# alekseyzimin/PacBio

Measured on NVIDIA B200. Metric: pacbio_bases_aligned_per_s, higher is better.
Workload: dtype int64+f64

## Files before the change

pacbio_b200/csrc/align.cu:

```cuda
#include "align.cuh"
#include "group.cuh"

#include <algorithm>
#include <cmath>
#include <cstdlib>
#include <cstring>
#include <memory>

namespace {

static int setup_final_rows(mr_context* ctx, mr_workspace& ws, uint64_t Sc, coords_soa& fin) {
  memset(&fin, 0, sizeof(fin));
  MR_TRY(ws.fin_i32.ensure(ctx, Sc * 4 * 5)); MR_TRY(ws.fin_u32.ensure(ctx, Sc * 4 * 8)); MR_TRY(ws.fin_f64.ensure(ctx, Sc * 8 * 3));
  MR_TRY(ws.fin_u64.ensure(ctx, Sc * 8 * 3)); MR_TRY(ws.fin_u8.ensure(ctx, Sc * 2));
  { int32_t* b = ws.fin_i32.as<int32_t>(); fin.rs = b; fin.re = b + Sc; fin.qs = b + 2 * Sc; fin.qe = b + 3 * Sc; fin.nb_mers = b + 4 * Sc; }
  { uint32_t* b = ws.fin_u32.as<uint32_t>(); fin.pb_cons = b; fin.sr_cons = b + Sc; fin.pb_cover = b + 2 * Sc; fin.sr_cover = b + 3 * Sc;
    fin.ql = b + 4 * Sc; fin.sr = b + 5 * Sc; fin.read = b + 6 * Sc; fin.info_len = b + 7 * Sc; }
  { double* b = ws.fin_f64.as<double>(); fin.stretch = b; fin.offset = b + Sc; fin.avg_err = b + 2 * Sc; }
  { uint64_t* b = ws.fin_u64.as<uint64_t>(); fin.info_off = b; fin.chain_pos = b + Sc; }
  { uint8_t* b = ws.fin_u8.as<uint8_t>(); fin.rn = b; fin.use_bwd = b + Sc; }
  return MR_OK;
}

static int setup_graph_nodes(mr_context* ctx, mr_workspace& ws, uint64_t Sc, graph_args& GA) {
// ... 370 lines not shown
    }
    if(kMulti || sz) __stcs(rec + g0 + j, out);
    __stcs(size + g0 + j, sz);
    if((!kMulti || (part_flags & 2)) && sz) ++nlist;
  }
  if(kMulti && !(part_flags & 1)) nlook = 0;
  nlook = __reduce_add_sync(MR_FULL_MASK, nlook); ntail = __reduce_add_sync(MR_FULL_MASK, ntail);
  nlist = __reduce_add_sync(MR_FULL_MASK, nlist); nbucket = __reduce_add_sync(MR_FULL_MASK, nbucket);
  if((threadIdx.x & 31) == 0) {
    if(nlook) atomicAdd(&looked, nlook);
    if(ntail) atomicAdd(&scanned, ntail);
    if(nlist) atomicAdd(&listed, nlist);
    if(nbucket) atomicAdd(&buckets, nbucket);
  }
  __syncthreads();
  if(threadIdx.x == 0) {
    if(looked) atomicAdd(n_lookups, (unsigned long long)looked);
    if(scanned) atomicAdd(n_tails, (unsigned long long)scanned);
    if(listed) atomicAdd(n_lists, (unsigned long long)listed);
    if(buckets) atomicAdd(n_buckets, (unsigned long long)buckets);
  }
}

__global__ void __launch_bounds__(256) read_threshold_kernel(const uint64_t* __restrict__ read_start, uint32_t nbits,
                                                              uint32_t* __restrict__ size, uint32_t* __restrict__ thr_out) {
  __shared__ uint32_t hist[2048];
  __shared__ uint64_t sw[8];
  __shared__ uint32_t sh_bin, sh_before, sh_count;
  const uint32_t r = blockIdx.x;
  const uint64_t rs = read_start[r];
  const uint32_t rlen = (uint32_t)(read_start[r + 1] - rs);
  uint32_t* sz = size + rs;
  if(threadIdx.x == 0) sh_count = 0;
  __syncthreads();
  uint32_t mine = 0;
  for(uint32_t i = threadIdx.x; i < rlen; i += 256) mine += sz[i] != 0;
  if(mine) atomicAdd(&sh_count, mine);
  __syncthreads();
  const uint32_t L = sh_count;
  const double   scaled = (double)L * 0.99;
  const uint32_t sum_thresh = (uint32_t)round(scaled);
  if(L == 0 || sum_thresh >= L) { if(threadIdx.x == 0) thr_out[r] = 0xffffffffu; return; }
  uint32_t kth = sum_thresh + 1, prefix = 0, remaining = nbits;
  while(remaining > 0) {
    const uint32_t d = remaining < 11 ? remaining : 11, shift = remaining - d;
    for(int i = threadIdx.x; i < 2048; i += 256) hist[i] = 0;
    __syncthreads();
    for(uint32_t i = threadIdx.x; i < rlen; i += 256) {
      const uint32_t v = sz[i];
      if(v != 0 && (remaining >= 32 || (v >> remaining) == prefix)) atomicAdd(&hist[(v >> shift) & ((1u << d) - 1)], 1u);
    }
    __syncthreads();
    uint32_t local[8], s = 0;
#pragma unroll
    for(int j = 0; j < 8; ++j) { local[j] = hist[threadIdx.x * 8 + j]; s += local[j]; }
    uint64_t total;
    uint32_t before = (uint32_t)prim::block_exclusive_scan_256(s, sw, total);
    if(before < kth && kth <= before + s) {
#pragma unroll
      for(int j = 0; j < 8; ++j) {
        if(kth <= before + local[j]) { sh_bin = threadIdx.x * 8 + j; sh_before = before; break; }
        before += local[j];
      }
    }
    __syncthreads();
    kth -= sh_before;
    prefix = (prefix << d) | sh_bin;
    remaining = shift;
    __syncthreads();
  }
  if(threadIdx.x == 0) thr_out[r] = prefix;
  for(uint32_t i = threadIdx.x; i < rlen; i += 256) if(sz[i] > prefix) sz[i] = 0;
}

__device__ __forceinline__ void emit_hit(const index_view& iv, uint32_t read, uint32_t pb_off, uint32_t sa_rank, bool minus,
                                         uint64_t slot, uint64_t* __restrict__ keys, uint64_t* __restrict__ pays,
                                         uint32_t& n_bad) {
  uint32_t sr, off;
  bool inside;
  if(iv.saloc) {
    const uint2 l = __ldg(iv.saloc + sa_rank);
    sr = l.x; off = l.y;
    inside = sr != 0xffffffffu;
  } else inside = index_locate(iv, __ldg(iv.sa + sa_rank), sr, off);
  if(inside) {
    const int32_t soff = minus ? -(int32_t)off : (int32_t)off;
    keys[slot] = ((uint64_t)read << 32) | (iv.sr_base + sr);
    pays[slot] = (uint64_t)pb_off | ((uint64_t)(uint32_t)soff << 32);
  } else {
    keys[slot] = ((uint64_t)read << 32) | iv.nseq_all;
    pays[slot] = 0;
    ++n_bad;
  }
}

__global__ void __launch_bounds__(kSeedThreads) tile_hits_kernel(const uint64_t* __restrict__ read_start,
                                                                  const uint32_t* __restrict__ tile_read, const uint32_t* __restrict__ tile_pos,
                                                                  const uint32_t* __restrict__ size, uint32_t* __restrict__ tile_hits,
                                                                  unsigned long long* __restrict__ overflow) {
  __shared__ uint64_t sw[8];
  const uint32_t r = tile_read[blockIdx.x];
  const uint64_t rs = read_start[r];
  const uint32_t rlen = (uint32_t)(read_start[r + 1] - rs);
  const uint32_t tpos = tile_pos[blockIdx.x];
  uint32_t s = 0;
#pragma unroll
  for(int it = 0; it < kTile / kSeedThreads; ++it) {
    const uint32_t pos = tpos + it * kSeedThreads + threadIdx.x;
    if(pos < rlen) s += __ldcs(size + rs + pos);
  }
  uint64_t total;
  (void)prim::block_exclusive_scan_256(s, sw, total);
  if(threadIdx.x == 0) {
    tile_hits[blockIdx.x] = total > 0xffffffffULL ? 0xffffffffu : (uint32_t)total;
    if(total > 0xffffffffULL) atomicAdd(overflow, 1ULL);
  }
}

template<bool kMulti>
__global__ void __launch_bounds__(kSeedThreads) expand_kernel(index_view iv, const index_view* __restrict__ more_views, uint32_t nparts,
                                                               uint64_t rec_stride, const uint64_t* __restrict__ read_start,
                                                               const uint32_t* __restrict__ tile_read, const uint32_t* __restrict__ tile_pos,
                                                               const uint4* __restrict__ rec, const uint32_t* __restrict__ size,
                                                               const uint64_t* __restrict__ tile_off,
                                                               uint64_t* __restrict__ keys, uint64_t* __restrict__ pays,
                                                               unsigned long long* __restrict__ n_invalid) {
  __shared__ uint64_t sw[8];
  __shared__ uint32_t s_off[kSeedThreads];
  __shared__ uint4    s_rec[kSeedThreads];
  uint64_t run = tile_off[blockIdx.x];
  if(tile_off[blockIdx.x + 1] == run) return;
  const uint32_t r = tile_read[blockIdx.x];
  const uint64_t rs = read_start[r];
  const uint32_t rlen = (uint32_t)(read_start[r + 1] - rs);
  const uint32_t tpos = tile_pos[blockIdx.x];
  uint32_t n_bad = 0;
  for(int it = 0; it < kTile / kSeedThreads; ++it) {
    const uint32_t pos = tpos + it * kSeedThreads + threadIdx.x;
    uint32_t sz = 0;
    uint4 rc = make_uint4(0, 0, 0, 0);
    if(pos < rlen) {
      sz = __ldcs(size + rs + pos);
      if(sz) rc = __ldcs(rec + rs + pos);
    }
    uint64_t in_iter;
    s_off[threadIdx.x] = (uint32_t)prim::block_exclusive_scan_256(sz, sw, in_iter);
    s_rec[threadIdx.x] = rc;
    __syncthreads();
    for(uint32_t h = threadIdx.x; h < (uint32_t)in_iter; h += kSeedThreads) {
      uint32_t lo = 0, hi = kSeedThreads;
      while(hi - lo > 1) { const uint32_t mid = (lo + hi) >> 1; if(s_off[mid] <= h) lo = mid; else hi = mid; }
      uint4 c = s_rec[lo];
      uint32_t j = h - s_off[lo];
      if(kMulti) {
        uint32_t part = 0;
        while(j >= c.y + c.w && part + 1 < nparts) {
          j -= c.y + c.w;
          ++part;
          c = __ldg(rec + part * rec_stride + rs + tpos + it * kSeedThreads + lo);
        }
        const bool minus = j >= c.y;
        emit_hit(part ? more_views[part - 1] : iv, r, tpos + it * kSeedThreads + lo + 1, minus ? c.z + (j - c.y) : c.x + j, minus,
                 run + h, keys, pays, n_bad);
        continue;
      }
      const bool minus = j >= c.y;
      emit_hit(iv, r, tpos + it * kSeedThreads + lo + 1, minus ? c.z + (j - c.y) : c.x + j, minus, run + h, keys, pays, n_bad);
    }
    run += in_iter;
    __syncthreads();
  }
  if(n_bad) atomicAdd(n_invalid, (unsigned long long)n_bad);
}

__global__ void __launch_bounds__(256) fine_windows_kernel(uint64_t S, survivors sv, const uint64_t* __restrict__ read_start, uint32_t kk,
                                                            uint64_t* __restrict__ wkey, uint32_t* __restrict__ wrow,
                                                            double* __restrict__ wbegin, double* __restrict__ wend,
                                                            uint32_t* __restrict__ gread, uint32_t* __restrict__ gsr, uint32_t* __restrict__ giter) {
  const uint64_t i = (uint64_t)blockIdx.x * blockDim.x + threadIdx.x;
  if(i >= S) return;
  const uint32_t read = sv.read[i], sr = sv.sr[i];
  const double stretch = sv.stretch[i], offset = sv.offset[i], err = sv.avg_err[i];
  const double rl = (double)(read_start[read + 1] - read_start[read]);
  const double s1 = stretch + offset;
  wbegin[i] = fmax(0.0, s1 - err);
  const double t = stretch * (double)sv.ql[i];
  const double e1 = t + offset;
  const double e2 = e1 + err;
  wend[i] = fmin(rl, e2 - (double)kk);
  wkey[i] = ((uint64_t)read << 32) | sr;
  wrow[i] = (uint32_t)i;
  gread[i] = read; gsr[i] = sr; giter[i] = sv.iter[i];
}

__global__ void __launch_bounds__(kSeedThreads) fine_seed_kernel(index_view iv, bool first_part, uint32_t kk, packed_reads bases,
// ... 556 lines not shown
    typedef void (*seed_fn)(index_view, uint32_t, packed_reads, const uint64_t*, const uint32_t*, const uint32_t*, const uint32_t*, uint32_t,
                            uint4*, uint32_t*, unsigned long long*, unsigned long long*, unsigned long long*, unsigned long long*);
    auto pick = [](bool multi, const index_view& v) -> seed_fn {
      const bool nibs = v.nib != nullptr, bytes = v.tail_bytes == 1;
      if(multi) return nibs ? (bytes ? seed_lookup_kernel<true, true, true> : seed_lookup_kernel<true, true, false>)
                            : (bytes ? seed_lookup_kernel<true, false, true> : seed_lookup_kernel<true, false, false>);
      return nibs ? (bytes ? seed_lookup_kernel<false, true, true> : seed_lookup_kernel<false, true, false>)
                  : (bytes ? seed_lookup_kernel<false, false, true> : seed_lookup_kernel<false, false, false>);
    };
    for(uint32_t part = 0; part < nparts; ++part) {
      l2_window(ctx, st, part ? idx->more[part - 1] : idx, true);
      const index_view& pv = idx->part_view(part);
      pick(nparts > 1, pv)<<<ntiles, kSeedThreads, 0, st>>>(pv, nparts == 1 ? 3u : ((part == 0 ? 1u : 0u) | (part + 1 == nparts ? 2u : 0u)),
                                                           d_bases, d_read_start, ws.tile_read.as<uint32_t>(), ws.tile_pos.as<uint32_t>(),
                                                           ws.tile_tbase.as<uint32_t>(), p->max_count > 0 ? (uint32_t)p->max_count : 0u,
                                                           ws.rec.as<uint4>() + part * rec_stride, ws.size.as<uint32_t>(), ctr + 0, ctr + 6, ctr + 9, ctr + 10);
      MR_LAUNCHED(ctx);
    }
    l2_window(ctx, st, idx, false);
    timer.next("count threshold");
    uint32_t nbits = 32;
    if(p->max_count > 1) { nbits = 0; while((1u << nbits) < (uint32_t)p->max_count) ++nbits; }
    else if(p->max_count == 1) nbits = 1;
    read_threshold_kernel<<<nreads, 256, 0, st>>>(d_read_start, nbits, ws.size.as<uint32_t>(), ws.thr.as<uint32_t>());
    MR_LAUNCHED(ctx);
  }
  timer.next("hit expansion");
  if(ntiles) {
    tile_hits_kernel<<<ntiles, kSeedThreads, 0, st>>>(d_read_start, ws.tile_read.as<uint32_t>(), ws.tile_pos.as<uint32_t>(),
                                                     ws.size.as<uint32_t>(), ws.tile_cand.as<uint32_t>(), ctr + 11);
    MR_LAUNCHED(ctx);
  }
  MR_TRY((prim::exclusive_scan<prim::ptr_in_u32, uint64_t>(ctx, prim::ptr_in_u32{ ws.tile_cand.as<uint32_t>() }, ntiles, ws.hit_off.as<uint64_t>(),
                                                           ws.scan_scratch, (uint64_t*)(ctr + 1))));
  if(ntiles) MR_CUDA(ctx, cudaMemcpyAsync(ws.hit_off.as<uint64_t>() + ntiles, ctr + 1, sizeof(uint64_t), cudaMemcpyDeviceToDevice, st));
  int sr_bits = 1;
  while((1ULL << sr_bits) <= (uint64_t)iv.nseq_all) ++sr_bits;
  MR_CUDA(ctx, cudaMemcpyAsync(h_ctr, ctr, 12 * sizeof(uint64_t), cudaMemcpyDeviceToHost, st));
  MR_CUDA(ctx, ctx->wait(st));
  if(h_ctr[11]) return ctx->fail(MR_ELIMIT, "mr_align_batch: 2^32 or more hits in one 1024-base tile; use --max-count");
  const uint64_t H = h_ctr[1];
  MR_TRACE_MSG("batch: %u reads, %llu bases, %llu lookups, %llu raw hits", nreads, (unsigned long long)T, (unsigned long long)h_ctr[0], (unsigned long long)H);
  res->view.n_kmers_looked_up = h_ctr[0];
  res->view.n_tail_entries = h_ctr[6];
  res->view.n_lists = h_ctr[9];
  res->view.n_buckets = h_ctr[10];
  static const uint64_t hit_limit = getenv("MR_MAX_HITS") ? strtoull(getenv("MR_MAX_HITS"), nullptr, 0) : (1ULL << 32);
  if(H >= hit_limit) return ctx->fail(MR_ELIMIT, "mr_align_batch: too many hits in one batch; use smaller batches");

  uint64_t G = 0, S = 0, cap = 0;
  const bool taps = ctx->keep_taps;
  uint64_t *skeys = nullptr, *spays = nullptr;
  chain_args A;
  memset(&A, 0, sizeof(A));
  if(H) {
    MR_TRY(ws.key0.ensure(ctx, (H + 2) * 8)); MR_TRY(ws.key1.ensure(ctx, (H + 2) * 8));
    MR_TRY(ws.pay0.ensure(ctx, (H + 2) * 8)); MR_TRY(ws.pay1.ensure(ctx, (H + 2) * 8));
    if(nparts == 1)
      expand_kernel<false><<<ntiles, kSeedThreads, 0, st>>>(iv, nullptr, 1, 0, d_read_start, ws.tile_read.as<uint32_t>(), ws.tile_pos.as<uint32_t>(),
                                                          ws.rec.as<uint4>(), ws.size.as<uint32_t>(), ws.hit_off.as<uint64_t>(),
                                                          ws.key0.as<uint64_t>(), ws.pay0.as<uint64_t>(), ctr + 2);
    else
      expand_kernel<true><<<ntiles, kSeedThreads, 0, st>>>(iv, idx->more_views.as<index_view>(), nparts, rec_stride, d_read_start,
                                                         ws.tile_read.as<uint32_t>(), ws.tile_pos.as<uint32_t>(),
                                                         ws.rec.as<uint4>(), ws.size.as<uint32_t>(), ws.hit_off.as<uint64_t>(),
                                                         ws.key0.as<uint64_t>(), ws.pay0.as<uint64_t>(), ctr + 2);
    MR_LAUNCHED(ctx);
    timer.next("group sort");
    static const bool read_sort_on = !(getenv("MR_READ_SORT") && atoi(getenv("MR_READ_SORT")) == 0);
    const bool read_sort = read_sort_on && group_sort_usable(sr_bits);
    uint64_t *alt_key, *alt_pay;
    if(read_sort) {
      MR_TRY(ws.head.ensure(ctx, H + 2));
      group_sort_args GS;
      GS.keys_in = ws.key0.as<uint64_t>(); GS.pays_in = ws.pay0.as<uint64_t>();
      GS.keys_out = ws.key1.as<uint64_t>(); GS.pays_out = ws.pay1.as<uint64_t>();
      GS.head = ws.head.as<uint8_t>(); GS.hit_off = ws.hit_off.as<uint64_t>(); GS.tile_first = ws.tile_first.as<uint32_t>();
      GS.nseq_all = iv.nseq_all; GS.sr_bits = sr_bits; GS.n_invalid_groups = ctr + 14; GS.cap = 0; GS.idx_bits = 0;
      MR_TRY(launch_group_sort(ctx, GS, nreads));
      skeys = GS.keys_out; spays = GS.pays_out; alt_key = GS.keys_in; alt_pay = GS.pays_in;
      MR_TRY((prim::flag_count<head_byte>(ctx, head_byte{ GS.head }, H, ws.scan_scratch, (uint64_t*)(ctr + 3))));
    } else {
      bool in_first = true;
      MR_TRY((prim::radix_sort_pairs<uint64_t, uint64_t>(ctx, ws.key0.as<uint64_t>(), ws.pay0.as<uint64_t>(), ws.key1.as<uint64_t>(),
                                                         ws.pay1.as<uint64_t>(), H, 0, sr_bits, ws.sort, &in_first)));
      skeys = in_first ? ws.key0.as<uint64_t>() : ws.key1.as<uint64_t>();
      spays = in_first ? ws.pay0.as<uint64_t>() : ws.pay1.as<uint64_t>();
      alt_key = in_first ? ws.key1.as<uint64_t>() : ws.key0.as<uint64_t>();
      alt_pay = in_first ? ws.pay1.as<uint64_t>() : ws.pay0.as<uint64_t>();
      MR_TRY((prim::flag_count<head_flag>(ctx, head_flag{ skeys, iv.nseq_all }, H, ws.scan_scratch, (uint64_t*)(ctr + 3))));
    }
    MR_CUDA(ctx, cudaMemcpyAsync(h_ctr, ctr, 16 * sizeof(uint64_t), cudaMemcpyDeviceToHost, st));
    MR_CUDA(ctx, ctx->wait(st));
    G = h_ctr[3];
    MR_TRACE_MSG("sorted (%s); %llu groups", read_sort ? "per read" : "device-wide", (unsigned long long)G);
    const uint64_t Hvalid = H - h_ctr[2];
    res->view.n_hits = Hvalid;
    res->view.n_groups = G - (read_sort ? h_ctr[14] : 0);
    MR_TRY(ws.group_start.ensure(ctx, (G + 2) * 8));
    if(read_sort) {
      MR_TRY((prim::flag_positions<head_byte>(ctx, head_byte{ ws.head.as<uint8_t>() }, H, ws.scan_scratch, ws.group_start.as<uint64_t>())));
      MR_CUDA(ctx, cudaMemcpyAsync(ws.group_start.as<uint64_t>() + G, ctr + 1, 8, cudaMemcpyDeviceToDevice, st));
// ... 563 lines not shown
```

pacbio_b200/csrc/align.cuh:

```cuda
#pragma once
#include <algorithm>
#include <cstdlib>
#include "index.cuh"
#include "primitives.cuh"

#include <mutex>

constexpr int      kTile        = 1024;
constexpr int      kSeedThreads = 256;
constexpr uint32_t kNone        = 0xffffffffu;

struct packed_reads {
  const uint64_t* __restrict__ codes;
  const uint64_t* __restrict__ nmask;
  int tma;
};

struct coords_soa {
  int32_t  *rs, *re, *qs, *qe, *nb_mers;
  uint32_t *pb_cons, *sr_cons, *pb_cover, *sr_cover, *ql, *sr, *read;
  uint8_t  *rn, *use_bwd;
  double   *stretch, *offset, *avg_err;
  uint64_t *info_off;
  uint32_t *info_len;
  uint64_t *chain_pos;
};

struct fine_buffers {
  dev_buf wkey0, wkey1, wrow0, wrow1, wbegin, wend, gread, gsr, giter, table_off, row_cnt, group_start;
  prim::sort_scratch sort;
};

struct mr_staged {
// ... 118 lines not shown
```

pacbio_b200/csrc/group.cu:

```cuda
#include "align.cuh"
#include "group.cuh"

namespace {

constexpr int kGsRounds  = 16;
constexpr int kGsDigit   = 7;
constexpr int kGsRadix   = 1 << kGsDigit;
constexpr int kFbRounds  = 4;

template<int kThreads>
struct gs_layout {
  static constexpr int kWarps = kThreads / 32;
  static constexpr int kCap   = kThreads * kGsRounds;
  static constexpr size_t pay_off = 0;
  static constexpr size_t arr_off = pay_off + (size_t)(kCap + 2) * 8;
  static constexpr size_t cnt_off = arr_off + (size_t)kCap * 4;
  static constexpr size_t tot_off = cnt_off + (size_t)kWarps * kGsRadix * 4;
  static constexpr size_t dbs_off = tot_off + kGsRadix * 4;
  static constexpr size_t bsz_off = dbs_off + kGsRadix * 4;
  static constexpr size_t bst_off = bsz_off + kGsRadix * 4;
  static constexpr size_t wsm_off = bst_off + kGsRadix * 4;
  static constexpr size_t cbs_off = wsm_off + 16;
  static constexpr size_t bar_off = cbs_off + kGsRadix * 4;
  static constexpr size_t bytes   = bar_off + 32;
// ... 59 lines not shown
  uint32_t run = 0, inc = 0;
  if(threadIdx.x < kGsRadix) {
#pragma unroll 8
    for(int w = 0; w < kWarps; ++w) { const uint32_t t = cnt[w][threadIdx.x]; cnt[w][threadIdx.x] = run; run += t; }
    tot[threadIdx.x] = run;
    if(kScan) {
      inc = run;
#pragma unroll
      for(int s = 1; s < 32; s <<= 1) { const uint32_t o = __shfl_up_sync(MR_FULL_MASK, inc, s); if(lane >= (unsigned)s) inc += o; }
      if(lane == 31) wsum[warp] = inc;
    }
  }
  __syncthreads();
  if(kScan) {
    if(threadIdx.x < kGsRadix) {
      uint32_t before = 0;
      for(unsigned w = 0; w < warp; ++w) before += wsum[w];
      dbase[threadIdx.x] = before + inc - run;
    }
    __syncthreads();
  }
}

template<int kThreads, bool kMatch>
__device__ void sort_range_smem(const uint64_t* kin, const uint64_t* pin, uint64_t* ko, uint64_t* po, uint8_t* head,
                                uint32_t n, uint32_t key_base, int key_bits, uint32_t ib, uint64_t rhi, uint32_t& phase) {
  typedef gs_sm<kThreads> Sm;
  constexpr int kWarps = kThreads / 32;
  const unsigned warp = threadIdx.x >> 5, lt = lanemask_lt();
  uint32_t* arr = Sm::arr();
  const uint32_t skew = (uint32_t)(((uintptr_t)pin >> 3) & 1u);
  if(threadIdx.x == 0) {
    const uint32_t bytes = ((n + skew + 1) & ~1u) * 8u;
    mbar_expect_tx(Sm::bar(), bytes);
    bulk_copy_g2s(Sm::spay(), pin - skew, bytes, Sm::bar());
  }
#pragma unroll 4
  for(uint32_t j = threadIdx.x; j < n; j += kThreads) arr[j] = (((uint32_t)kin[j] - key_base) << ib) | j;
  __syncthreads();
  const uint32_t R = (n + kThreads - 1) / kThreads;
  const uint32_t piece = warp * 32 * R + (threadIdx.x & 31);
  const int passes = (key_bits + kGsDigit - 1) / kGsDigit;
  for(int p = 0; p < passes; ++p) {
    const int shift = (int)ib + p * kGsDigit;
    for(int i = threadIdx.x; i < kWarps * kGsRadix; i += kThreads) (&Sm::cnt()[0][0])[i] = 0;
    __syncthreads();
    uint32_t e[kGsRounds], rk[kGsRounds / 2];
#pragma unroll
    for(int i = 0; i < kGsRounds; ++i) {
      if((i & 1) == 0) rk[i >> 1] = 0;
      if((uint32_t)i < R) {
        const uint32_t pos = piece + i * 32;
        const bool valid = pos < n;
        e[i] = valid ? arr[pos] : 0u;
        rk[i >> 1] |= rank_round<kMatch>(valid ? (e[i] >> shift) & (kGsRadix - 1) : (uint32_t)kGsRadix, Sm::cnt()[warp], lt) << (16 * (i & 1));
      }
    }
    __syncthreads();
    digit_prefix<kWarps, true>(Sm::cnt(), Sm::tot(), Sm::dbase(), Sm::wsum());
#pragma unroll
    for(int i = 0; i < kGsRounds; ++i) {
      if((uint32_t)i < R && piece + i * 32 < n) {
        const uint32_t d = (e[i] >> shift) & (kGsRadix - 1);
        arr[Sm::dbase()[d] + Sm::cnt()[warp][d] + ((rk[i >> 1] >> (16 * (i & 1))) & 0xffffu)] = e[i];
      }
    }
    __syncthreads();
  }
  mbar_wait(Sm::bar(), phase & 1u);
  ++phase;
  const uint32_t imask = (1u << ib) - 1;
#pragma unroll 4
  for(uint32_t j = threadIdx.x; j < n; j += kThreads) {
    const uint32_t x = arr[j], rel = x >> ib;
    ko[j] = rhi | (uint64_t)(key_base + rel);
    po[j] = Sm::spay()[skew + (x & imask)];
    head[j] = j == 0 || (arr[j - 1] >> ib) != rel;
  }
  __syncthreads();
}

template<int kThreads, bool kMatch>
__device__ void radix_pass_global(const uint64_t* sk, const uint64_t* sp, uint64_t* dk, uint64_t* dp, uint32_t n,
                                  int shift, uint32_t dmask, bool keep, uint32_t& gc) {
  typedef gs_sm<kThreads> Sm;
  constexpr int kWarps = kThreads / 32, kChunk = kThreads * kFbRounds;
  const unsigned lane = threadIdx.x & 31, warp = threadIdx.x >> 5, lt = lanemask_lt();
  uint32_t *tot = Sm::tot(), *gbase = Sm::dbase(), *cbase = Sm::cbase();
  uint16_t (*C)[kWarps][kGsRadix] = reinterpret_cast<uint16_t (*)[kWarps][kGsRadix]>(Sm::cnt());
  for(int i = threadIdx.x; i < kGsRadix; i += kThreads) tot[i] = 0;
  for(int i = threadIdx.x; i < kWarps * kGsRadix; i += kThreads) (&C[0][0][0])[i] = 0;
  asm volatile("fence.proxy.async;" ::: "memory");
  __syncthreads();
// ... 77 lines not shown
__device__ void sort_range_global(uint64_t* ak, uint64_t* ap, uint64_t* bk, uint64_t* bp, uint8_t* head,
                                  uint32_t n, int bits, bool stay, uint32_t& gc) {
  int passes = (bits + kGsDigit - 1) / kGsDigit;
  if(((passes & 1) == 0) != stay) ++passes;
  if(passes) {
    const int width = max(1, (bits + passes - 1) / passes);
    for(int p = 0; p < passes; ++p) {
      radix_pass_global<kThreads, kMatch>(ak, ap, bk, bp, n, p * width, (1u << width) - 1, false, gc);
      uint64_t* t = ak; ak = bk; bk = t;
      t = ap; ap = bp; bp = t;
    }
  }
  for(uint32_t j = threadIdx.x; j < n; j += kThreads) head[j] = j == 0 || (uint32_t)ak[j] != (uint32_t)ak[j - 1];
  __syncthreads();
}

template<int kThreads, bool kMatch>
__global__ void __launch_bounds__(kThreads, kThreads == 1024 ? 1 : 2) group_sort_kernel(group_sort_args A) {
  typedef gs_sm<kThreads> Sm;

  const uint32_t r = blockIdx.x;
  const uint64_t seg = A.hit_off[A.tile_first[r]];
  const uint64_t n64 = A.hit_off[A.tile_first[r + 1]] - seg;
  if(n64 == 0) return;
  const uint32_t n = (uint32_t)n64;
  const uint64_t rhi = (uint64_t)r << 32;
  uint32_t phase = 0, gc = 0;
  if(threadIdx.x == 0) { mbar_init(Sm::bar(), 1); mbar_init(Sm::cbar(), 1); mbar_init(Sm::cbar() + 1, 1); mbar_init(Sm::cbar() + 2, 1); }
  __syncthreads();
  uint64_t *kin = A.keys_in + seg, *pin = A.pays_in + seg, *ko = A.keys_out + seg, *po = A.pays_out + seg;
  uint8_t* head = A.head + seg;

  if(n <= A.cap) {
    sort_range_smem<kThreads, kMatch>(kin, pin, ko, po, head, n, 0u, A.sr_bits, A.idx_bits, rhi, phase);
  } else {
    const int low_bits = A.sr_bits > kGsDigit ? A.sr_bits - kGsDigit : 0;
    if(low_bits + (int)A.range_idx_bits > 32) {
      sort_range_global<kThreads, kMatch>(kin, pin, ko, po, head, n, A.sr_bits, false, gc);
    } else {
      radix_pass_global<kThreads, kMatch>(kin, pin, ko, po, n, low_bits, kGsRadix - 1, true, gc);
      asm volatile("fence.proxy.async;" ::: "memory");
      __syncthreads();
      const uint32_t rcap = A.range_cap;
      uint32_t b = 0;
      while(b < (uint32_t)kGsRadix) {
        const uint32_t sz = Sm::bsize()[b];
        if(sz == 0) { ++b; continue; }
        const uint32_t at = Sm::bstart()[b];
        if(sz > rcap) {
          sort_range_global<kThreads, kMatch>(ko + at, po + at, kin + at, pin + at, head + at, sz, low_bits, true, gc);
          asm volatile("fence.proxy.async;" ::: "memory");
          __syncthreads();
          ++b;
          continue;
        }
        uint32_t b1 = b + 1, total = sz;
        while(b1 < (uint32_t)kGsRadix) {
          const uint32_t nb = b1 + 1 - b;
          const int kb = low_bits + (32 - __clz(nb - 1));
          if(total + Sm::bsize()[b1] > rcap || kb + (int)A.range_idx_bits > 32) break;
          total += Sm::bsize()[b1];
          ++b1;
        }
        const uint32_t nb = b1 - b;
        const int kb = low_bits + (nb > 1 ? 32 - __clz(nb - 1) : 0);
        sort_range_smem<kThreads, kMatch>(ko + at, po + at, ko + at, po + at, head + at, total, b << low_bits, kb, A.range_idx_bits, rhi, phase);
        b = b1;
      }
    }
  }
  if(threadIdx.x == 0 && (uint32_t)ko[n - 1] == A.nseq_all) atomicAdd(A.n_invalid_groups, 1ULL);
}

}

int group_sort_threads() {
  static const int v = [] { const char* e = getenv("MR_GSORT_THREADS"); const int x = e ? atoi(e) : 0; return x == 1024 ? 1024 : 512; }();
  return v;
}

static int group_sort_cap_bits() {
  static const int env_bits = [] { const char* e = getenv("MR_GSORT_CAP"); int x = e ? atoi(e) : 0, b = 0; while((2 << b) <= x) ++b; return x >= 32 ? b : 31; }();
  return std::min(group_sort_threads() == 1024 ? 14 : 13, env_bits);
}

bool group_sort_usable(int sr_bits) {
  return std::max(0, sr_bits - kGsDigit) + group_sort_cap_bits() <= 32;
}

int launch_group_sort(mr_context* ctx, group_sort_args A, uint32_t nreads) {
  if(!nreads) return MR_OK;
  const int cb = group_sort_cap_bits();
  A.range_idx_bits = (uint32_t)cb; A.range_cap = 1u << cb;
  A.idx_bits = (uint32_t)std::max(0, std::min(cb, 32 - A.sr_bits));
  A.cap = A.sr_bits + 5 <= 32 ? 1u << A.idx_bits : 0u;
  typedef void (*kernel_t)(group_sort_args);
  const bool wide = group_sort_threads() == 1024;
  const kernel_t fn = wide ? (g_gs_match ? group_sort_kernel<1024, true> : group_sort_kernel<1024, false>)
                           : (g_gs_match ? group_sort_kernel<512, true> : group_sort_kernel<512, false>);
  const size_t smem = wide ? gs_layout<1024>::bytes : gs_layout<512>::bytes;
  MR_CUDA(ctx, cudaFuncSetAttribute(fn, cudaFuncAttributeMaxDynamicSharedMemorySize, (int)smem));
  fn<<<nreads, wide ? 1024 : 512, smem, ctx->stream>>>(A);
  MR_LAUNCHED(ctx);
  return MR_OK;
}
```

pacbio_b200/csrc/group.cuh:

```cuda
#pragma once
#include "common.cuh"

struct group_sort_args {
  uint64_t* keys_in;  uint64_t* pays_in;
  uint64_t* keys_out; uint64_t* pays_out;
  uint8_t*  head;
  const uint64_t* hit_off;
  const uint32_t* tile_first;
  uint32_t nseq_all;
  int      sr_bits;
  unsigned long long* n_invalid_groups;
  uint32_t cap, idx_bits, range_cap, range_idx_bits;
};

bool group_sort_usable(int sr_bits);
int launch_group_sort(mr_context* ctx, group_sort_args A, uint32_t nreads);
```

Measured before the change: 9.770 billion.

## Fuse hit expansion into per-read group sort and fold tile counts into thresholding

Tile hit counting moves into read_threshold_kernel, which now zeroes over-threshold sizes and writes per-tile totals plus a per-read max in the same pass, so the separate tile_hits_kernel goes away. For reads whose hit count fits the in-shared-memory cap, a new expand_group_kernel expands hits directly into shared memory and sorts them there, skipping the global key/pay write and re-read. The old expand_kernel and group_sort_kernel now run only for oversized reads, gated on a host-read max counter. This adds more kernel variants and shared-memory pressure, and the per-read loop in the threshold kernel serialises tile scans.

```diff
diff --git a/pacbio_b200/csrc/align.cu b/pacbio_b200/csrc/align.cu
--- a/pacbio_b200/csrc/align.cu
+++ b/pacbio_b200/csrc/align.cu
@@ -416,8 +416,10 @@
   }
 }
 
-__global__ void __launch_bounds__(256) read_threshold_kernel(const uint64_t* __restrict__ read_start, uint32_t nbits,
-                                                              uint32_t* __restrict__ size, uint32_t* __restrict__ thr_out) {
+__global__ void __launch_bounds__(256) read_threshold_kernel(const uint64_t* __restrict__ read_start, const uint32_t* __restrict__ tile_first,
+                                                              uint32_t nbits, uint32_t* __restrict__ size, uint32_t* __restrict__ thr_out,
+                                                              uint32_t* __restrict__ tile_hits, unsigned long long* __restrict__ overflow,
+                                                              unsigned long long* __restrict__ max_hits) {
   __shared__ uint32_t hist[2048];
   __shared__ uint64_t sw[8];
   __shared__ uint32_t sh_bin, sh_before, sh_count;
@@ -434,108 +436,87 @@
   const uint32_t L = sh_count;
   const double   scaled = (double)L * 0.99;
   const uint32_t sum_thresh = (uint32_t)round(scaled);
-  if(L == 0 || sum_thresh >= L) { if(threadIdx.x == 0) thr_out[r] = 0xffffffffu; return; }
-  uint32_t kth = sum_thresh + 1, prefix = 0, remaining = nbits;
-  while(remaining > 0) {
-    const uint32_t d = remaining < 11 ? remaining : 11, shift = remaining - d;
-    for(int i = threadIdx.x; i < 2048; i += 256) hist[i] = 0;
-    __syncthreads();
-    for(uint32_t i = threadIdx.x; i < rlen; i += 256) {
-      const uint32_t v = sz[i];
-      if(v != 0 && (remaining >= 32 || (v >> remaining) == prefix)) atomicAdd(&hist[(v >> shift) & ((1u << d) - 1)], 1u);
-    }
-    __syncthreads();
-    uint32_t local[8], s = 0;
+  uint32_t prefix = 0xffffffffu;
+  if(L != 0 && sum_thresh < L) {
+    uint32_t kth = sum_thresh + 1, remaining = nbits;
+    prefix = 0;
+    while(remaining > 0) {
+      const uint32_t d = remaining < 11 ? remaining : 11, shift = remaining - d;
+      for(int i = threadIdx.x; i < 2048; i += 256) hist[i] = 0;
+      __syncthreads();
+      for(uint32_t i = threadIdx.x; i < rlen; i += 256) {
+        const uint32_t v = sz[i];
+        if(v != 0 && (remaining >= 32 || (v >> remaining) == prefix)) atomicAdd(&hist[(v >> shift) & ((1u << d) - 1)], 1u);
+      }
+      __syncthreads();
+      uint32_t local[8], s = 0;
 #pragma unroll
-    for(int j = 0; j < 8; ++j) { local[j] = hist[threadIdx.x * 8 + j]; s += local[j]; }
+      for(int j = 0; j < 8; ++j) { local[j] = hist[threadIdx.x * 8 + j]; s += local[j]; }
+      uint64_t total;
+      uint32_t before = (uint32_t)prim::block_exclusive_scan_256(s, sw, total);
+      if(before < kth && kth <= before + s) {
+#pragma unroll
+        for(int j = 0; j < 8; ++j) {
+          if(kth <= before + local[j]) { sh_bin = threadIdx.x * 8 + j; sh_before = before; break; }
+          before += local[j];
+        }
+      }
+      __syncthreads();
+      kth -= sh_before;
+      prefix = (prefix << d) | sh_bin;
+      remaining = shift;
+      __syncthreads();
+    }
+  }
+  if(threadIdx.x == 0) thr_out[r] = prefix;
+  const uint32_t t0 = tile_first[r], nt = tile_first[r + 1] - t0;
+  uint64_t read_hits = 0;
+  for(uint32_t t = 0; t < nt; ++t) {
+    uint64_t s = 0;
+#pragma unroll
+    for(int it = 0; it < kTile / 256; ++it) {
+      const uint32_t i = t * kTile + it * 256 + threadIdx.x;
+      if(i < rlen) {
+        const uint32_t v = sz[i];
+        if(v > prefix) sz[i] = 0;
+        else s += v;
+      }
+    }
     uint64_t total;
-    uint32_t before = (uint32_t)prim::block_exclusive_scan_256(s, sw, total);
-    if(before < kth && kth <= before + s) {
-#pragma unroll
-      for(int j = 0; j < 8; ++j) {
-        if(kth <= before + local[j]) { sh_bin = threadIdx.x * 8 + j; sh_before = before; break; }
-        before += local[j];
-      }
-    }
-    __syncthreads();
-    kth -= sh_before;
-    prefix = (prefix << d) | sh_bin;
-    remaining = shift;
-    __syncthreads();
-  }
-  if(threadIdx.x == 0) thr_out[r] = prefix;
-  for(uint32_t i = threadIdx.x; i < rlen; i += 256) if(sz[i] > prefix) sz[i] = 0;
-}
-
-__device__ __forceinline__ void emit_hit(const index_view& iv, uint32_t read, uint32_t pb_off, uint32_t sa_rank, bool minus,
-                                         uint64_t slot, uint64_t* __restrict__ keys, uint64_t* __restrict__ pays,
-                                         uint32_t& n_bad) {
-  uint32_t sr, off;
-  bool inside;
-  if(iv.saloc) {
-    const uint2 l = __ldg(iv.saloc + sa_rank);
-    sr = l.x; off = l.y;
-    inside = sr != 0xffffffffu;
-  } else inside = index_locate(iv, __ldg(iv.sa + sa_rank), sr, off);
-  if(inside) {
-    const int32_t soff = minus ? -(int32_t)off : (int32_t)off;
-    keys[slot] = ((uint64_t)read << 32) | (iv.sr_base + sr);
-    pays[slot] = (uint64_t)pb_off | ((uint64_t)(uint32_t)soff << 32);
-  } else {
-    keys[slot] = ((uint64_t)read << 32) | iv.nseq_all;
-    pays[slot] = 0;
-    ++n_bad;
-  }
-}
-
-__global__ void __launch_bounds__(kSeedThreads) tile_hits_kernel(const uint64_t* __restrict__ read_start,
-                                                                  const uint32_t* __restrict__ tile_read, const uint32_t* __restrict__ tile_pos,
-                                                                  const uint32_t* __restrict__ size, uint32_t* __restrict__ tile_hits,
-                                                                  unsigned long long* __restrict__ overflow) {
-  __shared__ uint64_t sw[8];
-  const uint32_t r = tile_read[blockIdx.x];
-  const uint64_t rs = read_start[r];
-  const uint32_t rlen = (uint32_t)(read_start[r + 1] - rs);
-  const uint32_t tpos = tile_pos[blockIdx.x];
-  uint32_t s = 0;
-#pragma unroll
-  for(int it = 0; it < kTile / kSeedThreads; ++it) {
-    const uint32_t pos = tpos + it * kSeedThreads + threadIdx.x;
-    if(pos < rlen) s += __ldcs(size + rs + pos);
-  }
-  uint64_t total;
-  (void)prim::block_exclusive_scan_256(s, sw, total);
-  if(threadIdx.x == 0) {
-    tile_hits[blockIdx.x] = total > 0xffffffffULL ? 0xffffffffu : (uint32_t)total;
-    if(total > 0xffffffffULL) atomicAdd(overflow, 1ULL);
-  }
+    (void)prim::block_exclusive_scan_256(s, sw, total);
+    read_hits += total;
+    if(threadIdx.x == 0) {
+      tile_hits[t0 + t] = total > 0xffffffffULL ? 0xffffffffu : (uint32_t)total;
+      if(total > 0xffffffffULL) atomicAdd(overflow, 1ULL);
+    }
+  }
+  if(threadIdx.x == 0 && read_hits) atomicMax(max_hits, (unsigned long long)read_hits);
 }
 
 template<bool kMulti>
-__global__ void __launch_bounds__(kSeedThreads) expand_kernel(index_view iv, const index_view* __restrict__ more_views, uint32_t nparts,
-                                                               uint64_t rec_stride, const uint64_t* __restrict__ read_start,
+__global__ void __launch_bounds__(kSeedThreads) expand_kernel(hit_lists L, const uint32_t* __restrict__ tile_first, uint32_t cap,
                                                                const uint32_t* __restrict__ tile_read, const uint32_t* __restrict__ tile_pos,
-                                                               const uint4* __restrict__ rec, const uint32_t* __restrict__ size,
                                                                const uint64_t* __restrict__ tile_off,
-                                                               uint64_t* __restrict__ keys, uint64_t* __restrict__ pays,
-                                                               unsigned long long* __restrict__ n_invalid) {
+                                                               uint64_t* __restrict__ keys, uint64_t* __restrict__ pays) {
   __shared__ uint64_t sw[8];
   __shared__ uint32_t s_off[kSeedThreads];
   __shared__ uint4    s_rec[kSeedThreads];
   uint64_t run = tile_off[blockIdx.x];
   if(tile_off[blockIdx.x + 1] == run) return;
   const uint32_t r = tile_read[blockIdx.x];
-  const uint64_t rs = read_start[r];
-  const uint32_t rlen = (uint32_t)(read_start[r + 1] - rs);
+  if(tile_off[tile_first[r + 1]] - tile_off[tile_first[r]] <= cap) return;
+  const uint64_t rs = L.read_start[r];
+  const uint32_t rlen = (uint32_t)(L.read_start[r + 1] - rs);
   const uint32_t tpos = tile_pos[blockIdx.x];
+  const uint64_t khi = (uint64_t)r << 32;
   uint32_t n_bad = 0;
   for(int it = 0; it < kTile / kSeedThreads; ++it) {
     const uint32_t pos = tpos + it * kSeedThreads + threadIdx.x;
     uint32_t sz = 0;
     uint4 rc = make_uint4(0, 0, 0, 0);
     if(pos < rlen) {
-      sz = __ldcs(size + rs + pos);
-      if(sz) rc = __ldcs(rec + rs + pos);
+      sz = __ldcs(L.size + rs + pos);
+      if(sz) rc = __ldcs(L.rec + rs + pos);
     }
     uint64_t in_iter;
     s_off[threadIdx.x] = (uint32_t)prim::block_exclusive_scan_256(sz, sw, in_iter);
@@ -544,27 +525,24 @@
     for(uint32_t h = threadIdx.x; h < (uint32_t)in_iter; h += kSeedThreads) {
       uint32_t lo = 0, hi = kSeedThreads;
       while(hi - lo > 1) { const uint32_t mid = (lo + hi) >> 1; if(s_off[mid] <= h) lo = mid; else hi = mid; }
-      uint4 c = s_rec[lo];
-      uint32_t j = h - s_off[lo];
-      if(kMulti) {
-        uint32_t part = 0;
-        while(j >= c.y + c.w && part + 1 < nparts) {
-          j -= c.y + c.w;
-          ++part;
-          c = __ldg(rec + part * rec_stride + rs + tpos + it * kSeedThreads + lo);
-        }
-        const bool minus = j >= c.y;
-        emit_hit(part ? more_views[part - 1] : iv, r, tpos + it * kSeedThreads + lo + 1, minus ? c.z + (j - c.y) : c.x + j, minus,
-                 run + h, keys, pays, n_bad);
-        continue;
+      const uint32_t at = tpos + it * kSeedThreads + lo;
+      bool minus;
+      uint32_t part, sr;
+      uint64_t pay;
+      const uint32_t rank = list_entry<kMulti>(L, rs + at, s_rec[lo], h - s_off[lo], minus, part);
+      if(locate_hit(part ? L.more_views[part - 1] : L.iv, at + 1, rank, minus, sr, pay)) {
+        keys[run + h] = khi | sr;
+        pays[run + h] = pay;
+      } else {
+        keys[run + h] = khi | L.iv.nseq_all;
+        pays[run + h] = 0;
+        ++n_bad;
       }
-      const bool minus = j >= c.y;
-      emit_hit(iv, r, tpos + it * kSeedThreads + lo + 1, minus ? c.z + (j - c.y) : c.x + j, minus, run + h, keys, pays, n_bad);
     }
     run += in_iter;
     __syncthreads();
   }
-  if(n_bad) atomicAdd(n_invalid, (unsigned long long)n_bad);
+  if(n_bad) atomicAdd(L.n_invalid, (unsigned long long)n_bad);
 }
 
 __global__ void __launch_bounds__(256) fine_windows_kernel(uint64_t S, survivors sv, const uint64_t* __restrict__ read_start, uint32_t kk,
@@ -1167,15 +1145,11 @@
     uint32_t nbits = 32;
     if(p->max_count > 1) { nbits = 0; while((1u << nbits) < (uint32_t)p->max_count) ++nbits; }
     else if(p->max_count == 1) nbits = 1;
-    read_threshold_kernel<<<nreads, 256, 0, st>>>(d_read_start, nbits, ws.size.as<uint32_t>(), ws.thr.as<uint32_t>());
+    read_threshold_kernel<<<nreads, 256, 0, st>>>(d_read_start, ws.tile_first.as<uint32_t>(), nbits, ws.size.as<uint32_t>(), ws.thr.as<uint32_t>(),
+                                                  ws.tile_cand.as<uint32_t>(), ctr + 11, ctr + 8);
     MR_LAUNCHED(ctx);
   }
   timer.next("hit expansion");
-  if(ntiles) {
-    tile_hits_kernel<<<ntiles, kSeedThreads, 0, st>>>(d_read_start, ws.tile_read.as<uint32_t>(), ws.tile_pos.as<uint32_t>(),
-                                                     ws.size.as<uint32_t>(), ws.tile_cand.as<uint32_t>(), ctr + 11);
-    MR_LAUNCHED(ctx);
-  }
   MR_TRY((prim::exclusive_scan<prim::ptr_in_u32, uint64_t>(ctx, prim::ptr_in_u32{ ws.tile_cand.as<uint32_t>() }, ntiles, ws.hit_off.as<uint64_t>(),
                                                            ws.scan_scratch, (uint64_t*)(ctr + 1))));
   if(ntiles) MR_CUDA(ctx, cudaMemcpyAsync(ws.hit_off.as<uint64_t>() + ntiles, ctr + 1, sizeof(uint64_t), cudaMemcpyDeviceToDevice, st));
@@ -1201,28 +1175,33 @@
   if(H) {
     MR_TRY(ws.key0.ensure(ctx, (H + 2) * 8)); MR_TRY(ws.key1.ensure(ctx, (H + 2) * 8));
     MR_TRY(ws.pay0.ensure(ctx, (H + 2) * 8)); MR_TRY(ws.pay1.ensure(ctx, (H + 2) * 8));
-    if(nparts == 1)
-      expand_kernel<false><<<ntiles, kSeedThreads, 0, st>>>(iv, nullptr, 1, 0, d_read_start, ws.tile_read.as<uint32_t>(), ws.tile_pos.as<uint32_t>(),
-                                                          ws.rec.as<uint4>(), ws.size.as<uint32_t>(), ws.hit_off.as<uint64_t>(),
-                                                          ws.key0.as<uint64_t>(), ws.pay0.as<uint64_t>(), ctr + 2);
-    else
-      expand_kernel<true><<<ntiles, kSeedThreads, 0, st>>>(iv, idx->more_views.as<index_view>(), nparts, rec_stride, d_read_start,
-                                                         ws.tile_read.as<uint32_t>(), ws.tile_pos.as<uint32_t>(),
-                                                         ws.rec.as<uint4>(), ws.size.as<uint32_t>(), ws.hit_off.as<uint64_t>(),
-                                                         ws.key0.as<uint64_t>(), ws.pay0.as<uint64_t>(), ctr + 2);
-    MR_LAUNCHED(ctx);
-    timer.next("group sort");
+    hit_lists HL;
+    HL.iv = iv; HL.more_views = nparts > 1 ? idx->more_views.as<index_view>() : nullptr; HL.nparts = nparts; HL.rec_stride = rec_stride;
+    HL.read_start = d_read_start; HL.rec = ws.rec.as<uint4>(); HL.size = ws.size.as<uint32_t>(); HL.n_invalid = ctr + 2;
     static const bool read_sort_on = !(getenv("MR_READ_SORT") && atoi(getenv("MR_READ_SORT")) == 0);
     const bool read_sort = read_sort_on && group_sort_usable(sr_bits);
+    group_sort_args GS;
+    memset(&GS, 0, sizeof(GS));
+    if(read_sort) {
+      GS.keys_in = ws.key0.as<uint64_t>(); GS.pays_in = ws.pay0.as<uint64_t>();
+      GS.keys_out = ws.key1.as<uint64_t>(); GS.pays_out = ws.pay1.as<uint64_t>();
+      GS.hit_off = ws.hit_off.as<uint64_t>(); GS.tile_first = ws.tile_first.as<uint32_t>();
+      GS.nseq_all = iv.nseq_all; GS.sr_bits = sr_bits; GS.n_invalid_groups = ctr + 14;
+      group_sort_setup(GS);
+    }
+    const bool big_reads = h_ctr[8] > GS.cap;
+    if(big_reads) {
+      (nparts == 1 ? expand_kernel<false> : expand_kernel<true>)<<<ntiles, kSeedThreads, 0, st>>>(
+          HL, ws.tile_first.as<uint32_t>(), GS.cap, ws.tile_read.as<uint32_t>(), ws.tile_pos.as<uint32_t>(), ws.hit_off.as<uint64_t>(),
+          ws.key0.as<uint64_t>(), ws.pay0.as<uint64_t>());
+      MR_LAUNCHED(ctx);
+    }
+    timer.next("group sort");
     uint64_t *alt_key, *alt_pay;
     if(read_sort) {
       MR_TRY(ws.head.ensure(ctx, H + 2));
-      group_sort_args GS;
-      GS.keys_in = ws.key0.as<uint64_t>(); GS.pays_in = ws.pay0.as<uint64_t>();
-      GS.keys_out = ws.key1.as<uint64_t>(); GS.pays_out = ws.pay1.as<uint64_t>();
-      GS.head = ws.head.as<uint8_t>(); GS.hit_off = ws.hit_off.as<uint64_t>(); GS.tile_first = ws.tile_first.as<uint32_t>();
-      GS.nseq_all = iv.nseq_all; GS.sr_bits = sr_bits; GS.n_invalid_groups = ctr + 14; GS.cap = 0; GS.idx_bits = 0;
-      MR_TRY(launch_group_sort(ctx, GS, nreads));
+      GS.head = ws.head.as<uint8_t>();
+      MR_TRY(launch_group_sort(ctx, GS, HL, nreads, big_reads));
       skeys = GS.keys_out; spays = GS.pays_out; alt_key = GS.keys_in; alt_pay = GS.pays_in;
       MR_TRY((prim::flag_count<head_byte>(ctx, head_byte{ GS.head }, H, ws.scan_scratch, (uint64_t*)(ctr + 3))));
     } else {
diff --git a/pacbio_b200/csrc/align.cuh b/pacbio_b200/csrc/align.cuh
--- a/pacbio_b200/csrc/align.cuh
+++ b/pacbio_b200/csrc/align.cuh
@@ -9,6 +9,47 @@
 constexpr int      kTile        = 1024;
 constexpr int      kSeedThreads = 256;
 constexpr uint32_t kNone        = 0xffffffffu;
+
+
+struct hit_lists {
+  index_view iv;
+  const index_view* more_views;
+  uint32_t nparts;
+  uint64_t rec_stride;
+  const uint64_t* read_start;
+  const uint4* rec;
+  const uint32_t* size;
+  unsigned long long* n_invalid;
+};
+
+template<bool kMulti>
+__device__ __forceinline__ uint32_t list_entry(const hit_lists& L, uint64_t g, uint4 c, uint32_t j, bool& minus, uint32_t& part) {
+  part = 0;
+  if(kMulti) {
+    while(j >= c.y + c.w && part + 1 < L.nparts) {
+      j -= c.y + c.w;
+      ++part;
+      c = __ldg(L.rec + part * L.rec_stride + g);
+    }
+  }
+  minus = j >= c.y;
+  return minus ? c.z + (j - c.y) : c.x + j;
+}
+
+__device__ __forceinline__ bool locate_hit(const index_view& iv, uint32_t pb_off, uint32_t sa_rank, bool minus, uint32_t& sr, uint64_t& pay) {
+  uint32_t off;
+  bool inside;
+  if(iv.saloc) {
+    const uint2 l = __ldg(iv.saloc + sa_rank);
+    sr = l.x; off = l.y;
+    inside = sr != 0xffffffffu;
+  } else inside = index_locate(iv, __ldg(iv.sa + sa_rank), sr, off);
+  if(!inside) return false;
+  const int32_t soff = minus ? -(int32_t)off : (int32_t)off;
+  sr += iv.sr_base;
+  pay = (uint64_t)pb_off | ((uint64_t)(uint32_t)soff << 32);
+  return true;
+}
 
 struct packed_reads {
   const uint64_t* __restrict__ codes;
diff --git a/pacbio_b200/csrc/group.cu b/pacbio_b200/csrc/group.cu
--- a/pacbio_b200/csrc/group.cu
+++ b/pacbio_b200/csrc/group.cu
@@ -105,12 +105,9 @@
   }
 }
 
-template<int kThreads, bool kMatch>
-__device__ void sort_range_smem(const uint64_t* kin, const uint64_t* pin, uint64_t* ko, uint64_t* po, uint8_t* head,
-                                uint32_t n, uint32_t key_base, int key_bits, uint32_t ib, uint64_t rhi, uint32_t& phase) {
+template<int kThreads>
+__device__ uint32_t load_range_smem(const uint64_t* kin, const uint64_t* pin, uint32_t n, uint32_t key_base, uint32_t ib) {
   typedef gs_sm<kThreads> Sm;
-  constexpr int kWarps = kThreads / 32;
-  const unsigned warp = threadIdx.x >> 5, lt = lanemask_lt();
   uint32_t* arr = Sm::arr();
   const uint32_t skew = (uint32_t)(((uintptr_t)pin >> 3) & 1u);
   if(threadIdx.x == 0) {
@@ -121,6 +118,16 @@
 #pragma unroll 4
   for(uint32_t j = threadIdx.x; j < n; j += kThreads) arr[j] = (((uint32_t)kin[j] - key_base) << ib) | j;
   __syncthreads();
+  return skew;
+}
+
+template<int kThreads, bool kMatch>
+__device__ void sort_range_smem(uint64_t* ko, uint64_t* po, uint8_t* head, uint32_t n, uint32_t key_base, int key_bits,
+                                uint32_t ib, uint64_t rhi, uint32_t skew, uint32_t* phase) {
+  typedef gs_sm<kThreads> Sm;
+  constexpr int kWarps = kThreads / 32;
+  const unsigned warp = threadIdx.x >> 5, lt = lanemask_lt();
+  uint32_t* arr = Sm::arr();
   const uint32_t R = (n + kThreads - 1) / kThreads;
   const uint32_t piece = warp * 32 * R + (threadIdx.x & 31);
   const int passes = (key_bits + kGsDigit - 1) / kGsDigit;
@@ -150,8 +157,10 @@
     }
     __syncthreads();
   }
-  mbar_wait(Sm::bar(), phase & 1u);
-  ++phase;
+  if(phase) {
+    mbar_wait(Sm::bar(), *phase & 1u);
+    ++*phase;
+  }
   const uint32_t imask = (1u << ib) - 1;
 #pragma unroll 4
   for(uint32_t j = threadIdx.x; j < n; j += kThreads) {
@@ -275,7 +284,7 @@
   const uint32_t r = blockIdx.x;
   const uint64_t seg = A.hit_off[A.tile_first[r]];
   const uint64_t n64 = A.hit_off[A.tile_first[r + 1]] - seg;
-  if(n64 == 0) return;
+  if(n64 <= A.cap) return;
   const uint32_t n = (uint32_t)n64;
   const uint64_t rhi = (uint64_t)r << 32;
   uint32_t phase = 0, gc = 0;
@@ -284,45 +293,132 @@
   uint64_t *kin = A.keys_in + seg, *pin = A.pays_in + seg, *ko = A.keys_out + seg, *po = A.pays_out + seg;
   uint8_t* head = A.head + seg;
 
-  if(n <= A.cap) {
-    sort_range_smem<kThreads, kMatch>(kin, pin, ko, po, head, n, 0u, A.sr_bits, A.idx_bits, rhi, phase);
+  const int low_bits = A.sr_bits > kGsDigit ? A.sr_bits - kGsDigit : 0;
+  if(low_bits + (int)A.range_idx_bits > 32) {
+    sort_range_global<kThreads, kMatch>(kin, pin, ko, po, head, n, A.sr_bits, false, gc);
   } else {
-    const int low_bits = A.sr_bits > kGsDigit ? A.sr_bits - kGsDigit : 0;
-    if(low_bits + (int)A.range_idx_bits > 32) {
-      sort_range_global<kThreads, kMatch>(kin, pin, ko, po, head, n, A.sr_bits, false, gc);
-    } else {
-      radix_pass_global<kThreads, kMatch>(kin, pin, ko, po, n, low_bits, kGsRadix - 1, true, gc);
-      asm volatile("fence.proxy.async;" ::: "memory");
-      __syncthreads();
-      const uint32_t rcap = A.range_cap;
-      uint32_t b = 0;
-      while(b < (uint32_t)kGsRadix) {
-        const uint32_t sz = Sm::bsize()[b];
-        if(sz == 0) { ++b; continue; }
-        const uint32_t at = Sm::bstart()[b];
-        if(sz > rcap) {
-          sort_range_global<kThreads, kMatch>(ko + at, po + at, kin + at, pin + at, head + at, sz, low_bits, true, gc);
-          asm volatile("fence.proxy.async;" ::: "memory");
-          __syncthreads();
-          ++b;
-          continue;
+    radix_pass_global<kThreads, kMatch>(kin, pin, ko, po, n, low_bits, kGsRadix - 1, true, gc);
+    asm volatile("fence.proxy.async;" ::: "memory");
+    __syncthreads();
+    const uint32_t rcap = A.range_cap;
+    uint32_t b = 0;
+    while(b < (uint32_t)kGsRadix) {
+      const uint32_t sz = Sm::bsize()[b];
+      if(sz == 0) { ++b; continue; }
+      const uint32_t at = Sm::bstart()[b];
+      if(sz > rcap) {
+        sort_range_global<kThreads, kMatch>(ko + at, po + at, kin + at, pin + at, head + at, sz, low_bits, true, gc);
+        asm volatile("fence.proxy.async;" ::: "memory");
+        __syncthreads();
+        ++b;
+        continue;
+      }
+      uint32_t b1 = b + 1, total = sz;
+      while(b1 < (uint32_t)kGsRadix) {
+        const uint32_t nb = b1 + 1 - b;
+        const int kb = low_bits + (32 - __clz(nb - 1));
+        if(total + Sm::bsize()[b1] > rcap || kb + (int)A.range_idx_bits > 32) break;
+        total += Sm::bsize()[b1];
+        ++b1;
+      }
+      const uint32_t nb = b1 - b;
+      const int kb = low_bits + (nb > 1 ? 32 - __clz(nb - 1) : 0);
+      const uint32_t skew = load_range_smem<kThreads>(ko + at, po + at, total, b << low_bits, A.range_idx_bits);
+      sort_range_smem<kThreads, kMatch>(ko + at, po + at, head + at, total, b << low_bits, kb, A.range_idx_bits, rhi, skew, &phase);
+      b = b1;
+    }
+  }
+  if(threadIdx.x == 0 && (uint32_t)ko[n - 1] == A.nseq_all) atomicAdd(A.n_invalid_groups, 1ULL);
+}
+
+constexpr int kXHits = 4;
+template<int kThreads, bool kMatch, bool kMulti>
+__global__ void __launch_bounds__(kThreads, kThreads == 1024 ? 1 : 2) expand_group_kernel(group_sort_args A, hit_lists L) {
+  typedef gs_sm<kThreads> Sm;
+  constexpr int kWarps = kThreads / 32, kChunk = kWarps * kGsRadix, kPer = kChunk / kThreads;
+  static_assert(kPer == 4, "four positions per thread: one uint4 of offsets");
+  const uint32_t r = blockIdx.x;
+  const uint64_t seg = A.hit_off[A.tile_first[r]];
+  const uint64_t n64 = A.hit_off[A.tile_first[r + 1]] - seg;
+  if(n64 == 0 || n64 > A.cap) return;
+  const uint32_t n = (uint32_t)n64;
+  const uint64_t rs = L.read_start[r];
+  const uint32_t rlen = (uint32_t)(L.read_start[r + 1] - rs);
+  const unsigned lane = threadIdx.x & 31, warp = threadIdx.x >> 5;
+  const uint32_t ib = A.idx_bits;
+  uint32_t* off = &Sm::cnt()[0][0];
+  uint32_t* wtot = Sm::tot();
+  uint32_t nxt[kPer];
+#pragma unroll
+  for(int i = 0; i < kPer; ++i) { const uint32_t p = i * kThreads + threadIdx.x; nxt[i] = p < rlen ? __ldcs(L.size + rs + p) : 0u; }
+  uint32_t base = 0, n_bad = 0;
+  for(uint32_t c0 = 0; base < n && c0 < rlen; c0 += kChunk) {
+#pragma unroll
+    for(int i = 0; i < kPer; ++i) off[i * kThreads + threadIdx.x] = nxt[i];
+    __syncthreads();
+    const uint4 v = reinterpret_cast<const uint4*>(off)[threadIdx.x];
+#pragma unroll
+    for(int i = 0; i < kPer; ++i) {
+      const uint32_t p = c0 + kChunk + i * kThreads + threadIdx.x;
+      nxt[i] = p < rlen ? __ldcs(L.size + rs + p) : 0u;
+    }
+    const uint32_t own = v.x + v.y + v.z + v.w;
+    uint32_t inc = own;
+#pragma unroll
+    for(int d = 1; d < 32; d <<= 1) { const uint32_t o = __shfl_up_sync(MR_FULL_MASK, inc, d); if(lane >= (unsigned)d) inc += o; }
+    if(lane == 31) wtot[warp] = inc;
+    __syncthreads();
+    uint32_t before = 0, total = 0;
+#pragma unroll
+    for(int w = 0; w < kWarps; ++w) { const uint32_t x = wtot[w]; if((unsigned)w < warp) before += x; total += x; }
+    const uint32_t e = before + inc - own;
+    reinterpret_cast<uint4*>(off)[threadIdx.x] = make_uint4(e, e + v.x, e + v.x + v.y, e + v.x + v.y + v.z);
+    __syncthreads();
+    for(uint32_t h0 = 0; h0 < total; h0 += kThreads * kXHits) {
+      uint4 c[kXHits];
+      uint32_t at[kXHits], jl[kXHits];
+#pragma unroll
+      for(int u = 0; u < kXHits; ++u) {
+        const uint32_t h = h0 + u * kThreads + threadIdx.x;
+        at[u] = kNone;
+        if(h < total) {
+          uint32_t lo = 0, hi = kChunk;
+          while(hi - lo > 1) { const uint32_t mid = (lo + hi) >> 1; if(off[mid] <= h) lo = mid; else hi = mid; }
+          at[u] = c0 + lo;
+          jl[u] = h - off[lo];
+          c[u] = __ldg(L.rec + rs + at[u]);
         }
-        uint32_t b1 = b + 1, total = sz;
-        while(b1 < (uint32_t)kGsRadix) {
-          const uint32_t nb = b1 + 1 - b;
-          const int kb = low_bits + (32 - __clz(nb - 1));
-          if(total + Sm::bsize()[b1] > rcap || kb + (int)A.range_idx_bits > 32) break;
-          total += Sm::bsize()[b1];
-          ++b1;
+      }
+      uint32_t sr[kXHits];
+      uint64_t pay[kXHits];
+#pragma unroll
+      for(int u = 0; u < kXHits; ++u) {
+        if(at[u] != kNone) {
+          bool minus;
+          uint32_t part;
+          const uint32_t rank = list_entry<kMulti>(L, rs + at[u], c[u], jl[u], minus, part);
+          if(!locate_hit(part ? L.more_views[part - 1] : L.iv, at[u] + 1, rank, minus, sr[u], pay[u])) {
+            sr[u] = A.nseq_all;
+            pay[u] = 0;
+            ++n_bad;
+          }
         }
-        const uint32_t nb = b1 - b;
-        const int kb = low_bits + (nb > 1 ? 32 - __clz(nb - 1) : 0);
-        sort_range_smem<kThreads, kMatch>(ko + at, po + at, ko + at, po + at, head + at, total, b << low_bits, kb, A.range_idx_bits, rhi, phase);
-        b = b1;
-      }
-    }
-  }
-  if(threadIdx.x == 0 && (uint32_t)ko[n - 1] == A.nseq_all) atomicAdd(A.n_invalid_groups, 1ULL);
+      }
+#pragma unroll
+      for(int u = 0; u < kXHits; ++u) {
+        if(at[u] != kNone) {
+          const uint32_t j = base + h0 + u * kThreads + threadIdx.x;
+          Sm::spay()[j] = pay[u];
+          Sm::arr()[j] = (sr[u] << ib) | j;
+        }
+      }
+    }
+    base += total;
+    __syncthreads();
+  }
+  if(n_bad) atomicAdd(L.n_invalid, (unsigned long long)n_bad);
+  sort_range_smem<kThreads, kMatch>(A.keys_out + seg, A.pays_out + seg, A.head + seg, n, 0u, A.sr_bits, ib, (uint64_t)r << 32, 0u, nullptr);
+  if(threadIdx.x == 0 && (uint32_t)A.keys_out[seg + n - 1] == A.nseq_all) atomicAdd(A.n_invalid_groups, 1ULL);
 }
 
 }
@@ -341,19 +437,36 @@
   return std::max(0, sr_bits - kGsDigit) + group_sort_cap_bits() <= 32;
 }
 
-int launch_group_sort(mr_context* ctx, group_sort_args A, uint32_t nreads) {
-  if(!nreads) return MR_OK;
+void group_sort_setup(group_sort_args& A) {
   const int cb = group_sort_cap_bits();
   A.range_idx_bits = (uint32_t)cb; A.range_cap = 1u << cb;
   A.idx_bits = (uint32_t)std::max(0, std::min(cb, 32 - A.sr_bits));
   A.cap = A.sr_bits + 5 <= 32 ? 1u << A.idx_bits : 0u;
-  typedef void (*kernel_t)(group_sort_args);
+}
+
+int launch_group_sort(mr_context* ctx, const group_sort_args& A, const hit_lists& L, uint32_t nreads, bool big_reads) {
+  if(!nreads) return MR_OK;
   const bool wide = group_sort_threads() == 1024;
-  const kernel_t fn = wide ? (g_gs_match ? group_sort_kernel<1024, true> : group_sort_kernel<1024, false>)
-                           : (g_gs_match ? group_sort_kernel<512, true> : group_sort_kernel<512, false>);
   const size_t smem = wide ? gs_layout<1024>::bytes : gs_layout<512>::bytes;
-  MR_CUDA(ctx, cudaFuncSetAttribute(fn, cudaFuncAttributeMaxDynamicSharedMemorySize, (int)smem));
-  fn<<<nreads, wide ? 1024 : 512, smem, ctx->stream>>>(A);
-  MR_LAUNCHED(ctx);
+  const int threads = wide ? 1024 : 512;
+  if(A.cap) {
+    typedef void (*expand_t)(group_sort_args, hit_lists);
+    const bool multi = L.nparts > 1;
+    const expand_t fn = wide ? (g_gs_match ? (multi ? expand_group_kernel<1024, true, true> : expand_group_kernel<1024, true, false>)
+                                           : (multi ? expand_group_kernel<1024, false, true> : expand_group_kernel<1024, false, false>))
+                             : (g_gs_match ? (multi ? expand_group_kernel<512, true, true> : expand_group_kernel<512, true, false>)
+                                           : (multi ? expand_group_kernel<512, false, true> : expand_group_kernel<512, false, false>));
+    MR_CUDA(ctx, cudaFuncSetAttribute(fn, cudaFuncAttributeMaxDynamicSharedMemorySize, (int)smem));
+    fn<<<nreads, threads, smem, ctx->stream>>>(A, L);
+    MR_LAUNCHED(ctx);
+  }
+  if(big_reads) {
+    typedef void (*kernel_t)(group_sort_args);
+    const kernel_t fn = wide ? (g_gs_match ? group_sort_kernel<1024, true> : group_sort_kernel<1024, false>)
+                             : (g_gs_match ? group_sort_kernel<512, true> : group_sort_kernel<512, false>);
+    MR_CUDA(ctx, cudaFuncSetAttribute(fn, cudaFuncAttributeMaxDynamicSharedMemorySize, (int)smem));
+    fn<<<nreads, threads, smem, ctx->stream>>>(A);
+    MR_LAUNCHED(ctx);
+  }
   return MR_OK;
 }
diff --git a/pacbio_b200/csrc/group.cuh b/pacbio_b200/csrc/group.cuh
--- a/pacbio_b200/csrc/group.cuh
+++ b/pacbio_b200/csrc/group.cuh
@@ -1,5 +1,5 @@
 #pragma once
-#include "common.cuh"
+#include "align.cuh"
 
 struct group_sort_args {
   uint64_t* keys_in;  uint64_t* pays_in;
@@ -14,4 +14,5 @@
 };
 
 bool group_sort_usable(int sr_bits);
-int launch_group_sort(mr_context* ctx, group_sort_args A, uint32_t nreads);
+void group_sort_setup(group_sort_args& A);
+int launch_group_sort(mr_context* ctx, const group_sort_args& A, const hit_lists& L, uint32_t nreads, bool big_reads);
```

After: 9.640 billion (median of 6 runs). 0.987x the previous value.
